# second-state/qwen3_asr_rs

Hardware: NVIDIA H100
Metric: real-time factor (audio-sec/wall-sec) Qwen3-ASR-0.6B 30s clips (higher is better)
Workload: dtype f32 (bf16 weights, fp32-exact activations)

## Files before the change

qwen3_asr_rs_b200/csrc/decode_batch.cu:

```cuda
#include <algorithm>
#include "mega_common.cuh"

namespace asrb {

namespace megab {
using namespace mega;

static constexpr int MAXSPLIT = 32;
static constexpr int MAXROWS = 8;
static constexpr int ATT_SCRATCH = 4 * HD + NCONS_WARPS * 2 * HD + NCONS_WARPS * 4 + 8 + 8 + 2 * HD;

struct Params {
    const DecLayerW* layers;
    const bf16* lm_head;
    const bf16* embed;
    const float* final_norm;
    const float* rope_cos; const float* rope_sin;
    float eps;
    int L, H, QD, KVD, I, V, nkv;
    int nb;
    float* x;
    float* kcache; float* vcache; size_t cache_layer_stride, cache_seq_stride; int max_ctx;
    float* part_val; int* part_idx; int n_part;
    int* pos; int* done; int* next_id; int* ids_out; int* n_out; int max_new;
// ... 46 lines not shown
            const uint32_t xrow = xp + (uint32_t)sq * (H * 2) + (uint32_t)swz16(xc0 + 2 * ks + bhalf, sq & 7) * 16u;
            uint32_t b00, b01, b10, b11, b20, b21;
            ldsm_x4(xrow + (uint32_t)bpl * PSTR, b00, b01, b10, b11);
            ldsm_x2(xrow + 2u * PSTR, b20, b21);
            mma16816(acc[nt], a0, a1, a2, a3, b00, b01);
            mma16816(acc1[nt], a0, a1, a2, a3, b10, b11);
            mma16816(acc2[nt], a0, a1, a2, a3, b20, b21);
        }
    }
#pragma unroll
    for (int nt = 0; nt < NT; ++nt)
#pragma unroll
        for (int k = 0; k < 4; ++k) acc[nt][k] += acc1[nt][k] + acc2[nt][k];
}

static constexpr uint32_t SX_EMPTY = 0xFFFFFFFFu;
__device__ __forceinline__ void sx_store(uint32_t* p, float v) {
    uint32_t b = __float_as_uint(v);
    if (b == SX_EMPTY) b = 0x7FFFFFFFu;
    asm volatile("red.relaxed.gpu.global.and.b32 [%0], %1;" ::"l"(p), "r"(b) : "memory");
}
__device__ __forceinline__ uint4 sx_load4(const uint32_t* p) {
    uint4 v;
    asm volatile("ld.relaxed.gpu.global.v4.u32 {%0, %1, %2, %3}, [%4];" : "=r"(v.x), "=r"(v.y), "=r"(v.z), "=r"(v.w) : "l"(p) : "memory");
    return v;
}

__device__ __forceinline__ void head_norm_rope_b(const uint2* __restrict__ src, uint32_t tag, const float* __restrict__ nw,
                                                 float eps, const float* __restrict__ cs, const float* __restrict__ sn,
                                                 float* dst, int lane) {
    float v[4];
    ll_poll4(src + lane, 32, tag, v);
    const float ss = warp_sum(v[0] * v[0] + v[1] * v[1] + v[2] * v[2] + v[3] * v[3]);
    const float r = 1.0f / sqrtf(ss / 128.f + eps);
#pragma unroll
    for (int i = 0; i < 4; ++i) v[i] = (v[i] * r) * __ldg(nw + lane + 32 * i);
#pragma unroll
    for (int i = 0; i < 2; ++i) {
        const int d = lane + 32 * i;
        const float c = cs[d], s = sn[d];
        const float a = v[i], b = v[i + 2];
// ... 755 lines not shown
```

qwen3_asr_rs_b200/csrc/decode_mega.cu:

```cuda
#include "mega_common.cuh"

namespace asrb {

namespace mega {

struct Params {
    const DecLayerW* layers;
    const bf16* lm_head;
    const bf16* embed;
    const float* final_norm;
    const float* rope_cos; const float* rope_sin;
    float eps;
    int L, H, QD, KVD, I, V, nq, nkv, group;
    float* x;
    float* kcache; float* vcache; size_t cache_layer_stride; int max_ctx;
    int nsplit;
    float* part_val; int* part_idx;
    int* pos; int* done; int* next_id; int* ids_out; int* n_out; int max_new;
    unsigned* bar;
    uint2* qkv_ll; uint2* part_ll; uint2* attn_ll; uint2* x_ll; uint2* act_ll;
    long long* dbg;
};

static_assert(KV_KEYS * HD * 4 == SLOT_BYTES, "K / V tiles travel through the weight ring: one tile per slot");

template <int K>
__device__ __forceinline__ void load_xr(const float* xs, float (&xr)[K / 32], int lane) {
    const int sw = ((lane >> 2) & 1) * 4;
#pragma unroll
    for (int c = 0; c < K / 256; ++c) {
        const float4 a = *reinterpret_cast<const float4*>(xs + (c * 32 + lane) * 8 + sw);
        const float4 b = *reinterpret_cast<const float4*>(xs + (c * 32 + lane) * 8 + 4 - sw);
        xr[c * 8 + 0] = a.x; xr[c * 8 + 1] = a.y; xr[c * 8 + 2] = a.z; xr[c * 8 + 3] = a.w;
        xr[c * 8 + 4] = b.x; xr[c * 8 + 5] = b.y; xr[c * 8 + 6] = b.z; xr[c * 8 + 7] = b.w;
    }
// ... 94 lines not shown
}

__device__ __forceinline__ float warp_reduce8(const float (&a)[8], int lane) {
    const bool h16 = lane & 16, h8 = lane & 8, h4 = lane & 4;
    float k[4];
#pragma unroll
    for (int i = 0; i < 4; ++i) k[i] = (h16 ? a[4 + i] : a[i]) + __shfl_xor_sync(0xffffffffu, h16 ? a[i] : a[4 + i], 16);
    float m0 = (h8 ? k[2] : k[0]) + __shfl_xor_sync(0xffffffffu, h8 ? k[0] : k[2], 8);
    float m1 = (h8 ? k[3] : k[1]) + __shfl_xor_sync(0xffffffffu, h8 ? k[1] : k[3], 8);
    float v = (h4 ? m1 : m0) + __shfl_xor_sync(0xffffffffu, h4 ? m0 : m1, 4);
    v += __shfl_xor_sync(0xffffffffu, v, 2);
    v += __shfl_xor_sync(0xffffffffu, v, 1);
    return v;
}

enum { ME_STORE = 0, ME_RESID = 1, ME_SWIGLU = 2, ME_ARGMAX = 3 };

template <int K>
__device__ __forceinline__ void consume_ksplit(const Slice& s, const Ring& ring, uint32_t& q, const float* xs, uint2* out,
                                               uint32_t tag, float* xres, float* part) {
    const int tid = threadIdx.x, lane = tid & 31, warp = tid >> 5;
    constexpr int NU = K / 8;
    constexpr int J = (NU + NCONS - 1) / NCONS;
    uint32_t grp = 0;
    for (int r = s.r0; r < s.r1;) {
        const int rowsA = min(s.rpc, s.r1 - r);
        const uint32_t slotA = q % ring.nslot;
        mbar_wait(&ring.full[slotA], (q / ring.nslot) & 1);
        const bool pair = s.rpc < 8 && r + rowsA < s.r1;
        const int rowsB = pair ? min(s.rpc, s.r1 - r - rowsA) : 0;
        const uint32_t slotB = (q + 1) % ring.nslot;
        if (pair) mbar_wait(&ring.full[slotB], ((q + 1) / ring.nslot) & 1);
        const uint4* baseA = reinterpret_cast<const uint4*>(ring.slots + (size_t)slotA * SLOT_BYTES);
        const uint4* baseB = reinterpret_cast<const uint4*>(ring.slots + (size_t)slotB * SLOT_BYTES);
        const int R = rowsA + rowsB;
// ... 29 lines not shown
            }
            const float v = warp_reduce8(acc, lane);
            if (g0 + 8 >= R) {
                __syncwarp();
                if (lane == 0) { mbar_arrive(&ring.empty[slotA]); if (pair) mbar_arrive(&ring.empty[slotB]); }
            }
            float* pb = part + (grp & 1) * 64;
            if ((lane & 3) == 0) pb[warp * 8 + (lane >> 2)] = v;
            cons_sync();
            if (tid < ng) {
                float t = pb[tid];
#pragma unroll
                for (int w8 = 1; w8 < NCONS_WARPS; ++w8) t += pb[w8 * 8 + tid];
                const int row = r + g0 + tid;
                const float nv = xres[row - s.r0] + t; xres[row - s.r0] = nv;
                ll_store(out + row, nv, tag);
            }
        }
        r += R; q += pair ? 2 : 1;
    }
}

template <int K, int EPI>
__device__ __forceinline__ void consume_quad(const Slice& s, const Ring& ring, uint32_t& q, const float* xs, uint2* out,
                                             uint32_t tag, float& best_v, int& best_i,
                                             const float* norm_w, float norm_r, long long* fine) {
    const int lane = threadIdx.x & 31, warp = threadIdx.x >> 5;
    int fi = 0;
#define CF() do { if (fine && threadIdx.x == 0 && fi < 24) fine[fi++] = clock64(); } while (0)
    CF();
    constexpr int NU = K / 8;
    float xr[K / 32];
    if (norm_w) load_xr_norm<K>(xs, norm_w, norm_r, xr, lane);
    else load_xr<K>(xs, xr, lane);
    cons_sync();
    CF();
    const int j = lane >> 3;
    for (int r = s.r0; r < s.r1;) {
        const int rowsA = min(s.rpc, s.r1 - r);
// ... 7 lines not shown
        const uint4* baseA = reinterpret_cast<const uint4*>(ring.slots + (size_t)slotA * SLOT_BYTES);
        const uint4* baseB = reinterpret_cast<const uint4*>(ring.slots + (size_t)slotB * SLOT_BYTES);
        const int R = rowsA + rowsB;
        for (int i0 = 4 * warp; i0 < R; i0 += 4 * NCONS_WARPS) {
            const int nv = min(4, R - i0);
            const uint4* rp[4];
#pragma unroll
            for (int i = 0; i < 4; ++i) {
                const int ri = i0 + (i < nv ? i : 0);
                rp[i] = ri < rowsA ? baseA + (size_t)ri * NU : baseB + (size_t)(ri - rowsA) * NU;
            }
            const float v = row_dot4<K>(rp[0], rp[1], rp[2], rp[3], xr, lane);
            const int row = r + i0 + j;
            if (EPI == ME_SWIGLU) {
                const float up = __shfl_xor_sync(0xffffffffu, v, 8);
                if ((lane & 15) == 0 && j < nv) ll_store(out + (row >> 1), silu(v) * up, tag);
            } else if (EPI == ME_STORE) {
                if ((lane & 7) == 0 && j < nv) ll_store(out + row, v, tag);
            } else {
                if ((lane & 7) == 0 && j < nv && v > best_v) { best_v = v; best_i = row; }
            }
        }
        CF();
        __syncwarp();
        if (lane == 0) { mbar_arrive(&ring.empty[slotA]); if (pair) mbar_arrive(&ring.empty[slotB]); }
        r += R; q += pair ? 2 : 1;
    }
    CF();
#undef CF
}

template <int K, int EPI>
__device__ __forceinline__ void consume(const Slice& s, const Ring& ring, uint32_t& q, const float* xs, uint2* out,
                                        uint32_t tag, float* xres, float& best_v, int& best_i,
                                        const float* norm_w = nullptr, float norm_r = 1.f, long long* fine = nullptr,
                                        float* part = nullptr) {
    if constexpr (EPI == ME_RESID) { consume_ksplit<K>(s, ring, q, xs, out, tag, xres, part); return; }
    else if constexpr (K <= 1024) { consume_quad<K, EPI>(s, ring, q, xs, out, tag, best_v, best_i, norm_w, norm_r, fine); return; }
    const int lane = threadIdx.x & 31, warp = threadIdx.x >> 5;
    int fi = 0;
#define CF() do { if (fine && threadIdx.x == 0 && fi < 24) fine[fi++] = clock64(); } while (0)
    CF();
    constexpr int RSTEP = (EPI == ME_SWIGLU) ? 2 : 1;
    constexpr bool XREG = K <= 2048;
    constexpr bool DUAL = XREG && K <= 1024;
    constexpr int KX = XREG ? K : 256;
    constexpr int UPW = (DUAL && EPI != ME_SWIGLU) ? 2 : 1;
    const int sub = lane >> 4;
    float xr[XREG ? K / 32 : 1];
    if (XREG) {
        if (norm_w) load_xr_norm<KX>(xs, norm_w, norm_r, reinterpret_cast<float (&)[KX / 32]>(xr), lane);
        else load_xr<KX>(xs, reinterpret_cast<float (&)[KX / 32]>(xr), lane);
        cons_sync();
// ... 11 lines not shown
        for (int ub = first * UPW; ub < units_here; ub += NCONS_WARPS * UPW) {
            if (EPI == ME_SWIGLU) {
                const int row = r + ub * 2;
                float v0, v1;
                if (DUAL) {
                    const float v = row_dot2<KX>(base + (size_t)(ub * 2) * (K / 8), base + (size_t)(ub * 2 + 1) * (K / 8),
                                                 reinterpret_cast<const float (&)[KX / 32]>(xr), lane);
                    v0 = v; v1 = __shfl_xor_sync(0xffffffffu, v, 16);
                } else if (XREG) {
                    v0 = row_dot<KX>(base + (size_t)(ub * 2) * (K / 8), reinterpret_cast<const float (&)[KX / 32]>(xr), lane);
                    v1 = row_dot<KX>(base + (size_t)(ub * 2 + 1) * (K / 8), reinterpret_cast<const float (&)[KX / 32]>(xr), lane);
                } else {
                    v0 = row_dot_smem<K>(base + (size_t)(ub * 2) * (K / 8), xs, lane);
                    v1 = row_dot_smem<K>(base + (size_t)(ub * 2 + 1) * (K / 8), xs, lane);
                }
                if (lane == 0) ll_store(out + (row >> 1), silu(v0) * v1, tag);
            } else {
                bool act; int row; float v0;
                if (DUAL) {
                    const bool two = ub + 1 < units_here;
                    v0 = row_dot2<KX>(base + (size_t)ub * (K / 8), base + (size_t)(two ? ub + 1 : ub) * (K / 8),
                                      reinterpret_cast<const float (&)[KX / 32]>(xr), lane);
                    act = ((lane & 15) == 0) && (sub == 0 || two);
                    row = r + ub + sub;
                } else {
                    if (XREG) v0 = row_dot<KX>(base + (size_t)ub * (K / 8), reinterpret_cast<const float (&)[KX / 32]>(xr), lane);
                    else v0 = row_dot_smem<K>(base + (size_t)ub * (K / 8), xs, lane);
                    act = lane == 0; row = r + ub;
                }
                if (EPI == ME_STORE) {
                    if (act) ll_store(out + row, v0, tag);
                } else if (EPI == ME_RESID) {
                    if (act) { const float nv = xres[row - s.r0] + v0; xres[row - s.r0] = nv; ll_store(out + row, nv, tag); }
                } else {
                    if (act && v0 > best_v) { best_v = v0; best_i = row; }
                }
            }
        }
        unit += (units_here + UPW - 1) / UPW * UPW;
        CF();
        __syncwarp();
        if (lane == 0) mbar_arrive(&ring.empty[slot]);
    }
    CF();
#undef CF
    if (!XREG) cons_sync();
}

// ... 34 lines not shown
#define MEGA_GT(k)                                                                                     \
    do {                                                                                               \
        if (p.dbg && tid == 0 && l == 5) {                                                             \
            unsigned long long t_; asm volatile("mov.u64 %0, %%globaltimer;" : "=l"(t_));               \
            p.dbg[512 + 3 * blockIdx.x + (k)] = (long long)t_;                                         \
        }                                                                                              \
    } while (0)
#define MEGA_MARK()                                                                                    \
    do {                                                                                               \
        if (dbg_row && tid == 0 && dbg_i < DBG_SLOTS) dbg_row[dbg_i++] = clock64();                    \
    } while (0)

template <int H, int QD, int I, int NS>
__global__ void __launch_bounds__(NTHREADS, 1) decode_step_kernel(const Params p) {
    constexpr int XS_FLOATS = (I > XS_MIN ? I : XS_MIN) + 64;
    extern __shared__ __align__(128) uint8_t smem[];
    constexpr int PARAM_FLOATS = 2 * H + 2 * HD;
    Ring ring;
    ring.slots = smem;
    ring.nslot = NS;
    float* xs = reinterpret_cast<float*>(smem + (size_t)NS * SLOT_BYTES);
    float* xres = xs + XS_FLOATS;
    float* pbuf = xres + XRES_MAX;
    float* ropes = pbuf + 2 * PARAM_FLOATS;
    DecLayerW* ltab = reinterpret_cast<DecLayerW*>(ropes + 128);
    uint64_t* bars = reinterpret_cast<uint64_t*>(ltab + MAX_LAYERS);
    ring.full = bars; ring.empty = bars + NSLOT_MAX;
    uint64_t* p_full = bars + 2 * NSLOT_MAX; uint64_t* p_empty = p_full + 2;
    float* red = reinterpret_cast<float*>(bars + 2 * NSLOT_MAX + 4);
    int* ired = reinterpret_cast<int*>(red + 64);
// ... 71 lines not shown

    long long* dbg_row = nullptr; int dbg_i = 0;
    if (p.dbg && (blockIdx.x == 0 || blockIdx.x == gridDim.x - 1)) dbg_row = p.dbg + (blockIdx.x == 0 ? 0 : DBG_SLOTS);
    MEGA_MARK();
    const int half = HD / 2;
    const float* cs = ropes;
    const float* sn = ropes + half;
    const unsigned G = gridDim.x;
    float best_v = -INFINITY; int best_i = 0x7fffffff;
    const unsigned epoch = __ldcg(p.bar + 1);
    const uint32_t tag_base = (epoch & 0xffffffu) << 8;
    const Slice xsl = make_slice(nullptr, H, QD, 1);
    Slice sl_qkv = make_slice(nullptr, QD + 2 * p.KVD, H, 1), sl_o = make_slice(nullptr, H, QD, 1),
          sl_gu = make_slice(nullptr, 2 * I, H, 2), sl_dn = make_slice(nullptr, H, I, 1);
    for (int i = tid; i < xsl.r1 - xsl.r0; i += NCONS) xres[i] = __ldcg(p.x + xsl.r0 + i);

    for (int l = 0; l < p.L; ++l) {
        const DecLayerW w = ltab[l];
        const uint32_t tl = tag_base | ((uint32_t)l << 3);
        const float* pb = pbuf + (l & 1) * PARAM_FLOATS;
        mbar_wait(&p_full[l & 1], (l >> 1) & 1);
        float nr;
        {
            float ss = 0.f;
            if (l == 0) { for (int i = tid; i < H; i += NCONS) { const float v = __ldcg(p.x + i); xs[xs_swz(i)] = v; ss = fmaf(v, v, ss); } }
            else { MEGA_FINE(0); MEGA_FINE(1); ss = ll_gather(p.x_ll, H, (tag_base | ((uint32_t)(l - 1) << 3)) | PH_XD, xs); MEGA_FINE(2); }
            nr = norm_scale(ss, H, p.eps, red);
            MEGA_FINE(3);
        }
        consume<H, ME_STORE>(sl_qkv, ring, q, xs, p.qkv_ll, tl | PH_QKV, xres, best_v, best_i, pb, nr);
        MEGA_FINE(4);
        MEGA_GT(0);
        MEGA_MARK();
        {
            const int nloc = n_old;
            const int nact = min(p.nsplit, (pos + KV_KEYS - 1) / KV_KEYS);
            const bool merger = att_cta && att_sp == 0;
            if (nloc > 0) {
                const int g = att_g;
                float* qs = xs;
                float* kn = qs + p.group * HD;
                float* vn = kn + HD;
                float* sc = vn + HD;
                float* ml = sc + p.group * KV_KEYS;
                float* osum = ml + 8;
// ... 176 lines not shown
                            ok = __all_sync(0xffffffffu, (mv.y == tg) && (lv.y == tg) && round_ok(0));
                        } while (!ok);
                        MEGA_FINE(35);
                        const float m_l = lane < nact ? __uint_as_float(mv.x) : (lane == nact ? snew[hq] : -INFINITY);
                        const float l_l = lane < nact ? __uint_as_float(lv.x) : (lane == nact ? 1.f : 0.f);
                        const float M = warp_max(m_l);
                        const float f = expf(m_l - M);
                        const float Lsum = warp_sum(f * l_l);
                        float O = __shfl_sync(0xffffffffu, f, nact) * vn[d];
                        for (int u0 = 0; u0 < nact; u0 += RB) {
                            if (u0 > 0) { do { load_round(u0); ok = __all_sync(0xffffffffu, round_ok(u0)); } while (!ok); }
#pragma unroll
                            for (int u = 0; u < RB; ++u)
                                if (u0 + u < nact) O = fmaf(__shfl_sync(0xffffffffu, f, u0 + u), __uint_as_float(ov[u].x), O);
                        }
                        ll_store(p.attn_ll + (size_t)(g * p.group + hq) * HD + d, O / Lsum, tl | PH_ATTN);
                    }
                }
                MEGA_FINE(31);
                cons_sync();
            }
        }
        MEGA_MARK();
        MEGA_FINE(32);
        ll_gather(p.attn_ll, QD, tl | PH_ATTN, xs);
        MEGA_FINE(33);
        MEGA_GT(2);
        cons_sync();
        consume<QD, ME_RESID>(sl_o, ring, q, xs, p.x_ll, tl | PH_XO, xres, best_v, best_i, nullptr, 1.f, nullptr, part);
        MEGA_FINE(34);
        MEGA_MARK();
        cons_sync();
        {
            MEGA_FINE(8); MEGA_FINE(9);
            const float ss = ll_gather(p.x_ll, H, tl | PH_XO, xs); MEGA_FINE(10);
            nr = norm_scale(ss, H, p.eps, red); MEGA_FINE(11);
        }
        consume<H, ME_SWIGLU>(sl_gu, ring, q, xs, p.act_ll, tl | PH_ACT, xres, best_v, best_i, pb + H, nr, (dbg_row && l == 5) ? dbg_row + 440 : nullptr);
        MEGA_FINE(12);
        MEGA_FINE(13);
        MEGA_MARK();
        MEGA_FINE(16); MEGA_FINE(17);
        ll_gather(p.act_ll, I, tl | PH_ACT, xs); MEGA_FINE(18);
        cons_sync();
        consume<I, ME_RESID>(sl_dn, ring, q, xs, p.x_ll, tl | PH_XD, xres, best_v, best_i, nullptr, 1.f, nullptr, part);
        MEGA_FINE(19);
        MEGA_FINE(20);
        MEGA_MARK();
        cons_sync();
        if (lane == 0) mbar_arrive(&p_empty[l & 1]);
    }
    float nrf;
    {
        const float ss = ll_gather(p.x_ll, H, (tag_base | ((uint32_t)(p.L - 1) << 3)) | PH_XD, xs);
        mbar_wait(&p_full[p.L & 1], (p.L >> 1) & 1);
        nrf = norm_scale(ss, H, p.eps, red);
    }
    consume<H, ME_ARGMAX>(make_slice(p.lm_head, p.V, H, 1), ring, q, xs, nullptr, 0u, xres, best_v, best_i,
                          pbuf + (p.L & 1) * PARAM_FLOATS, nrf);
    MEGA_MARK();
#pragma unroll
    for (int o = 8; o <= 16; o <<= 1) {
        const float ov = __shfl_xor_sync(0xffffffffu, best_v, o); const int oi = __shfl_xor_sync(0xffffffffu, best_i, o);
        if (ov > best_v || (ov == best_v && oi < best_i)) { best_v = ov; best_i = oi; }
    }
    cons_sync();
    if (lane == 0) { red[warp] = best_v; ired[warp] = best_i; }
    cons_sync();
    int& is_last = ired[63];
    if (tid == 0) {
        float v = -INFINITY; int idx = 0x7fffffff;
        for (int wq = 0; wq < NCONS_WARPS; ++wq)
            if (red[wq] > v || (red[wq] == v && ired[wq] < idx)) { v = red[wq]; idx = ired[wq]; }
// ... 17 lines not shown
            if (ov > v || (ov == v && oi < idx)) { v = ov; idx = oi; }
        }
        if (lane == 0) { red[warp] = v; ired[warp] = idx; }
        cons_sync();
        int& tok_s = ired[62];
        if (tid == 0) {
            for (int wq = 1; wq < NCONS_WARPS; ++wq)
                if (red[wq] > v || (red[wq] == v && ired[wq] < idx)) { v = red[wq]; idx = ired[wq]; }
            int tok = idx;
            const int n = *p.n_out;
            if (tok == 151643 || tok == 151645 || n >= p.max_new) { *p.done = 1; *p.next_id = -1; tok = -1; }
            else { p.ids_out[n] = tok; *p.n_out = n + 1; *p.pos = pos + 1; *p.next_id = tok; }
            tok_s = tok;
            p.bar[0] = 0;
            p.bar[1] = p.bar[1] + 1;
        }
        cons_sync();
        const int tok = tok_s;
        if (tok >= 0) {
            const bf16* e = p.embed + (size_t)tok * H;
            for (int i = tid; i < H; i += NCONS) p.x[i] = __bfloat162float(e[i]);
        }
    }
}

}

static long long* g_last_dbg = nullptr;

static int mega_xs_floats(int I) { return std::max(I, mega::XS_MIN) + 64; }
// ... 14 lines not shown
    if (B < 1 || c.head_dim != 128) return false;
    const int group = c.num_attention_heads / c.num_key_value_heads;
    if (group + 2 > mega::NCONS_WARPS) return false;
    if ((size_t)(group * 128 + 256 + group * mega::KV_KEYS + 8 + mega::NCONS_WARPS * 2 * 128 + mega::NCONS_WARPS * 4 + 8) > (size_t)mega_xs_floats(c.intermediate_size)) return false;
    if (m.ctx->smem_optin < mega_smem_bytes(c.hidden_size, c.intermediate_size, mega_nslot(c))) return false;
    if ((c.hidden_size + m.ctx->sm_count - 1) / m.ctx->sm_count + 1 > mega::XRES_MAX) return false;
    if (c.num_hidden_layers > 32) return false;
    if ((max_ctx + mega::KV_KEYS - 1) / mega::KV_KEYS > mega::MAX_SPLITS) return false;
    if (((max_ctx + mega::KV_KEYS - 1) / mega::KV_KEYS) * c.num_key_value_heads > m.ctx->sm_count) return false;
    return dims_match<1024, 2048, 3072>(c) || dims_match<2048, 2048, 6144>(c) || dims_match<256, 512, 512>(c);
}

size_t decode_mega_part_floats(const Model& m) {
    const asrb_dims& c = m.d.c;
    const int group = c.num_attention_heads / c.num_key_value_heads;
    const size_t words = (size_t)m.d.qkv_dim + (size_t)m.ctx->sm_count * group * mega::PSTRIDE + m.d.q_dim + c.hidden_size +
                         c.intermediate_size + 64;
    return 2 * words + 64;
}

void launch_decode_step_mega(const Model& m, const DecodeBufs& b, int B, float* kcache, float* vcache,
                             size_t cache_layer_stride, size_t cache_seq_stride, int max_ctx, int ctx_now, const MegaBufs& mb,
                             cudaStream_t st, int64_t* launches) {
    ASRB_REQUIRE(decode_mega_supported(m, B, ctx_now), ASRB_ERR_STATE, "fused decode step not supported for this model/batch/context");
    ASRB_REQUIRE(m.d_dec_layers && mb.bar && mb.part, ASRB_ERR_STATE, "fused decode step buffers missing");
    const asrb_dims& c = m.d.c;
    const int G = m.ctx->sm_count;
    const int group = c.num_attention_heads / c.num_key_value_heads;
    const int nsplit = std::min(mega::MAX_SPLITS, std::min(G / c.num_key_value_heads, (max_ctx + mega::KV_KEYS - 1) / mega::KV_KEYS));
    const size_t smem = mega_smem_bytes(c.hidden_size, c.intermediate_size, mega_nslot(c));
    const void* fn = nullptr;
    if (dims_match<1024, 2048, 3072>(c)) fn = (const void*)mega::decode_step_kernel<1024, 2048, 3072, 6>;
    else if (dims_match<2048, 2048, 6144>(c)) fn = (const void*)mega::decode_step_kernel<2048, 2048, 6144, 5>;
    else fn = (const void*)mega::decode_step_kernel<256, 512, 512, 6>;
    ASRB_CUDA_CHECK(cudaFuncSetAttribute(fn, cudaFuncAttributeMaxDynamicSharedMemorySize, (int)smem));
    for (int sb = 0; sb < B; ++sb) {
        mega::Params p{};
        p.layers = m.d_dec_layers; p.lm_head = m.lm_head; p.embed = m.embed; p.final_norm = m.final_norm_sw;
        p.rope_cos = m.rope_cos; p.rope_sin = m.rope_sin; p.eps = (float)c.rms_norm_eps;
        p.L = c.num_hidden_layers; p.H = c.hidden_size; p.QD = m.d.q_dim; p.KVD = m.d.kv_dim; p.I = c.intermediate_size;
        p.V = c.vocab_size; p.nq = c.num_attention_heads; p.nkv = c.num_key_value_heads; p.group = group;
        p.x = b.x + (size_t)sb * c.hidden_size;
        p.kcache = kcache + (size_t)sb * cache_seq_stride; p.vcache = vcache + (size_t)sb * cache_seq_stride;
        p.cache_layer_stride = cache_layer_stride; p.max_ctx = max_ctx; p.nsplit = nsplit;
        p.part_val = b.part_val; p.part_idx = b.part_idx;
        p.pos = b.pos + sb; p.done = b.done + sb; p.next_id = b.next_id + sb;
        p.ids_out = b.ids_out + (size_t)sb * b.max_new; p.n_out = b.n_out + sb; p.max_new = b.max_new;
        p.bar = mb.bar;
        uint2* w = reinterpret_cast<uint2*>(mb.part);
        p.qkv_ll = w; w += m.d.qkv_dim;
        p.part_ll = w; w += (size_t)G * group * mega::PSTRIDE;
        p.attn_ll = w; w += m.d.q_dim;
        p.x_ll = w; w += c.hidden_size;
        p.act_ll = w; w += c.intermediate_size;
        p.dbg = mb.dbg;
        g_last_dbg = mb.dbg;
        if (mb.steps_issued && ++*mb.steps_issued >= 0xFFFF00u) {
            ASRB_CUDA_CHECK(cudaMemsetAsync(mb.part, 0, mb.part_bytes, st));
            const unsigned one = 1;
            ASRB_CUDA_CHECK(cudaMemcpyAsync(mb.bar + 1, &one, sizeof(one), cudaMemcpyHostToDevice, st));
            *mb.steps_issued = 1;
        }
        void* args[] = {(void*)&p};
        ASRB_CUDA_CHECK(cudaLaunchCooperativeKernel(fn, dim3(G), dim3(mega::NTHREADS), args, smem, st));
        if (launches) *launches += 1;
    }
}

int decode_mega_debug_timeline(long long* out, int cap) {
// ... 9 lines not shown
```

qwen3_asr_rs_b200/csrc/internal.h:

```cpp
#pragma once
#include <atomic>
#include <map>
#include <string>
#include <vector>
#include "../../include/asr_b200.h"
#include "common.cuh"

namespace asrb {

struct Dims {
    asrb_dims c;
    int enc_hd;
    int chunk_frames;
    int chunks_per_window;
    int conv_h[4];
    int conv_w[4];
    int tok_per_chunk;
    int cpad;
    int feat;
    int q_dim, kv_dim, qkv_dim;
    void derive();
};
void validate_dims(const asrb_dims& d);
inline int conv_out_len(int l) { return (l - 1) / 2 + 1; }
// ... 121 lines not shown
    float* attn;
    float* act;
    float* logits;
    float* part_val; int* part_idx; int n_part;
    int* pos;
    int* done;
    int* next_id;
    int* ids_out;
    int* n_out;
    int max_new;
};
void launch_decode_step_phases(const Model& m, const DecodeBufs& b, int B, float* kcache, float* vcache,
                               size_t cache_layer_stride, size_t cache_seq_stride, int max_ctx,
                               bool write_logits, cudaStream_t st, int64_t* launches);
struct MegaBufs { unsigned* bar = nullptr; float* part = nullptr; long long* dbg = nullptr; size_t part_bytes = 0; unsigned* steps_issued = nullptr;
                  uint32_t* sx = nullptr; size_t sx_bytes = 0; int* sx_nb = nullptr; };
size_t decode_mega_part_floats(const Model& m);
size_t decode_batch_part_floats(const Model& m);
size_t decode_batch_sx_bytes(const Model& m);
bool decode_batch_supported(const Model& m, int B, int ctx);
int decode_mega_dbg_slots();
void launch_greedy(const Model& m, const DecodeBufs& b, int B, cudaStream_t st, int64_t* launches);
void launch_lmhead_argmax(const Model& m, const float* x_rows, const int* d_row_idx, int B,
                          const DecodeBufs& b, bool write_logits, cudaStream_t st, int64_t* launches);

}
```

qwen3_asr_rs_b200/csrc/mega_common.cuh:

```cuda
#pragma once
#include "internal.h"

namespace asrb {
namespace mega {

static constexpr int NCONS_WARPS = 8;
static constexpr int NCONS = NCONS_WARPS * 32;
static constexpr int NTHREADS = NCONS + 32;
static constexpr int SLOT_BYTES = 32 * 1024;
static constexpr int NSLOT_MAX = 6;
static constexpr int KV_KEYS = 64;
static constexpr int XS_MIN = 3072;
static constexpr int XRES_MAX = 64;
static constexpr int MAX_LAYERS = 32;
static constexpr int HD = 128;
static constexpr int PSTRIDE = HD + 2;
static constexpr int DBG_SLOTS = 1024;
static constexpr int MAX_SPLITS = 18;

enum { PH_QKV = 1, PH_PART = 2, PH_ATTN = 3, PH_XO = 4, PH_ACT = 5, PH_XD = 6 };

__device__ __forceinline__ uint32_t smem_u32(const void* p) { return (uint32_t)__cvta_generic_to_shared(p); }
__device__ __forceinline__ void mbar_init(uint64_t* bar, uint32_t count) {
    asm volatile("mbarrier.init.shared::cta.b64 [%0], %1;" ::"r"(smem_u32(bar)), "r"(count));
}
__device__ __forceinline__ void mbar_expect_tx(uint64_t* bar, uint32_t bytes) {
    asm volatile("mbarrier.arrive.expect_tx.shared::cta.b64 _, [%0], %1;" ::"r"(smem_u32(bar)), "r"(bytes) : "memory");
}
__device__ __forceinline__ void mbar_arrive(uint64_t* bar) {
    asm volatile("mbarrier.arrive.shared::cta.b64 _, [%0];" ::"r"(smem_u32(bar)) : "memory");
}
__device__ __forceinline__ void mbar_wait(uint64_t* bar, uint32_t parity) {
    asm volatile(
        "{\n"
        ".reg .pred p;\n"
// ... 11 lines not shown
__device__ __forceinline__ uint64_t l2_evict_first_policy() {
    uint64_t pol;
    asm volatile("createpolicy.fractional.L2::evict_first.b64 %0, 1.0;" : "=l"(pol));
    return pol;
}
__device__ __forceinline__ void bulk_g2s_hint(void* dst, const void* src, uint32_t bytes, uint64_t* bar, uint64_t pol) {
    asm volatile("cp.async.bulk.shared::cluster.global.mbarrier::complete_tx::bytes.L2::cache_hint [%0], [%1], %2, [%3], %4;"
                 ::"r"(smem_u32(dst)), "l"(src), "r"(bytes), "r"(smem_u32(bar)), "l"(pol) : "memory");
}
__device__ __forceinline__ void cons_sync() { asm volatile("bar.sync 1, %0;" ::"n"(NCONS) : "memory"); }

__device__ __forceinline__ void ll_store(uint2* p, float v, uint32_t tag) {
    const unsigned long long val = ((unsigned long long)tag << 32) | (unsigned long long)__float_as_uint(v);
    asm volatile("red.relaxed.gpu.global.max.u64 [%0], %1;" ::"l"(p), "l"(val) : "memory");
}
__device__ __forceinline__ uint4 ll_load2(const uint2* p) {
    uint4 v;
    asm volatile("ld.relaxed.gpu.global.v4.u32 {%0, %1, %2, %3}, [%4];" : "=r"(v.x), "=r"(v.y), "=r"(v.z), "=r"(v.w) : "l"(p) : "memory");
    return v;
}
__device__ __forceinline__ float ll_poll1(const uint2* p, uint32_t tag) {
    uint2 v;
    do {
        asm volatile("ld.relaxed.gpu.global.v2.u32 {%0, %1}, [%2];" : "=r"(v.x), "=r"(v.y) : "l"(p) : "memory");
    } while (v.y != tag);
    return __uint_as_float(v.x);
}
__device__ __forceinline__ void ll_poll4(const uint2* p, int stride, uint32_t tag, float (&out)[4]) {
    uint2 v[4];
    bool ok;
    do {
#pragma unroll
        for (int i = 0; i < 4; ++i)
            asm volatile("ld.relaxed.gpu.global.v2.u32 {%0, %1}, [%2];" : "=r"(v[i].x), "=r"(v[i].y) : "l"(p + (size_t)i * stride) : "memory");
        ok = (v[0].y == tag) && (v[1].y == tag) && (v[2].y == tag) && (v[3].y == tag);
    } while (!ok);
#pragma unroll
    for (int i = 0; i < 4; ++i) out[i] = __uint_as_float(v[i].x);
}
__device__ __forceinline__ int xs_swz(int e) { const int k = e >> 2; return ((k ^ ((k >> 3) & 1)) << 2) | (e & 3); }
__device__ __forceinline__ float ll_gather(const uint2* buf, int n, uint32_t tag, float* xs) {
    float ss = 0.f;
    const int pairs = n >> 1;
    constexpr int U = 8;
    for (int i0 = threadIdx.x; i0 < pairs; i0 += U * NCONS) {
        uint4 v[U];
#pragma unroll
        for (int u = 0; u < U; ++u) v[u] = make_uint4(0u, 0u, 0u, 0u);
        bool ok;
        do {
            ok = true;
#pragma unroll
            for (int u = 0; u < U; ++u) {
                const int i = i0 + u * NCONS;
                if (i < pairs && !(v[u].y == tag && v[u].w == tag)) v[u] = ll_load2(buf + 2 * i);
            }
#pragma unroll
            for (int u = 0; u < U; ++u) {
                const int i = i0 + u * NCONS;
                if (i < pairs) ok = ok && (v[u].y == tag) && (v[u].w == tag);
            }
        } while (!ok);
#pragma unroll
        for (int u = 0; u < U; ++u) {
            const int i = i0 + u * NCONS;
            if (i < pairs) {
                const float a = __uint_as_float(v[u].x), b = __uint_as_float(v[u].z);
                *reinterpret_cast<float2*>(xs + xs_swz(2 * i)) = make_float2(a, b);
                ss = fmaf(a, a, ss); ss = fmaf(b, b, ss);
            }
        }
    }
    return ss;
}

struct Ring {
    uint8_t* slots; uint64_t* full; uint64_t* empty;
    uint32_t nslot;
};

struct Slice { const bf16* W; int K, r0, r1, rpc; };
__device__ __forceinline__ Slice make_slice(const bf16* W, int N, int K, int rstep) {
// ... 12 lines not shown
```

qwen3_asr_rs_b200/csrc/session.cu:

```cuda
#include <algorithm>
#include <cstring>
#include "internal.h"

namespace asrb {

void model_set_tensor(Model* m, const char* name, int dtype, const int64_t* shape, int ndim, const void* host);
void model_finalize(Model* m);
struct IngestState;
IngestState* ingest_state_new();
void ingest_state_free(IngestState* st);
void ingest_pcm(IngestState* st, cudaStream_t stream, const void* const* pcm, const int64_t* n_frames, const int32_t* channels,
                const int32_t* rate, const int32_t* format, int batch, float* d_samples, int64_t max_samples_per_utt,
                int64_t* n_out, int64_t* soff_out);

static const int kPromptHead[9] = {151644, 8948, 198, 151645, 198, 151644, 872, 198, 151669};
static const int kPromptTail[6] = {151670, 151645, 198, 151644, 77091, 198};
static const int kAudioPad = 151676;

struct Session {
    Model* m = nullptr;
    cudaStream_t st = nullptr;
    int max_batch = 0, max_lang = 0, max_new = 0;
    int64_t max_samples = 0, max_npad = 0;
    int maxF = 0, maxC = 0, maxT = 0, maxS = 0, max_ctx = 0;
// ... 126 lines not shown
        b.act = salloc<float>(s, Bm * c.intermediate_size);
        b.logits = salloc<float>(s, Bm * c.vocab_size);
        b.n_part = m->ctx->sm_count * 2;
        b.part_val = salloc<float>(s, Bm * b.n_part);
        b.part_idx = salloc<int>(s, Bm * b.n_part);
        b.pos = salloc<int>(s, Bm); b.done = salloc<int>(s, Bm); b.next_id = salloc<int>(s, Bm);
        b.ids_out = salloc<int>(s, Bm * max_new); b.n_out = salloc<int>(s, Bm);
        b.max_new = max_new;
        s->d_lastrow = salloc<int>(s, Bm);
        s->mega.bar = salloc<unsigned>(s, 4, true);
        { const unsigned one = 1; ASRB_CUDA_CHECK(cudaMemcpy(s->mega.bar + 1, &one, sizeof(one), cudaMemcpyHostToDevice)); }
        const size_t part_floats = std::max(decode_mega_part_floats(*m), decode_batch_part_floats(*m));
        s->mega.part = salloc<float>(s, part_floats, true);
        s->mega.part_bytes = part_floats * sizeof(float);
        s->mega.steps_issued = &s->mega_steps;
        if (max_batch >= 2) {
            s->mega.sx_bytes = decode_batch_sx_bytes(*m);
            s->mega.sx = (uint32_t*)salloc<uint8_t>(s, s->mega.sx_bytes);
            ASRB_CUDA_CHECK(cudaMemset(s->mega.sx, 0xFF, s->mega.sx_bytes));
            s->mega.sx_nb = &s->sx_nb;
            int maxwin = 0, maxpersist = 0;
            cudaDeviceGetAttribute(&maxwin, cudaDevAttrMaxAccessPolicyWindowSize, m->ctx->device);
            cudaDeviceGetAttribute(&maxpersist, cudaDevAttrMaxPersistingL2CacheSize, m->ctx->device);
            if (maxwin > 0 && maxpersist > 0) {
                const size_t want = std::min<size_t>({s->mega.sx_bytes, (size_t)maxwin, (size_t)maxpersist});
                if (cudaDeviceSetLimit(cudaLimitPersistingL2CacheSize, want) == cudaSuccess) {
                    cudaStreamAttrValue av{};
                    av.accessPolicyWindow.base_ptr = s->mega.sx; av.accessPolicyWindow.num_bytes = want;
                    av.accessPolicyWindow.hitRatio = 1.0f; av.accessPolicyWindow.hitProp = cudaAccessPropertyPersisting;
                    av.accessPolicyWindow.missProp = cudaAccessPropertyStreaming;
// ... 429 lines not shown
```

Before: 294.6.

## Replace tagged LL buffers in single-sequence mega decode with per-layer sentinel exchange buffers

The single-sequence fused decode kernel stops exchanging attention output, residual and activations through tagged 64-bit LL slots. It now uses per-layer, double-buffered 32-bit sentinel buffers (all-ones means empty) that are filled with atomic AND and polled with vectorized relaxed loads. Because the buffers are distinct per layer, several cons_sync barriers between phases are removed, and the k-split residual now writes straight into these buffers. Each step clears the other parity's buffers, which adds global stores. The exchange also halves its traffic per value and uses a new gather pattern, optionally as a noinline call when H > 1024.

```diff
diff --git a/qwen3_asr_rs_b200/csrc/decode_batch.cu b/qwen3_asr_rs_b200/csrc/decode_batch.cu
--- a/qwen3_asr_rs_b200/csrc/decode_batch.cu
+++ b/qwen3_asr_rs_b200/csrc/decode_batch.cu
@@ -84,17 +84,6 @@
         for (int k = 0; k < 4; ++k) acc[nt][k] += acc1[nt][k] + acc2[nt][k];
 }
 
-static constexpr uint32_t SX_EMPTY = 0xFFFFFFFFu;
-__device__ __forceinline__ void sx_store(uint32_t* p, float v) {
-    uint32_t b = __float_as_uint(v);
-    if (b == SX_EMPTY) b = 0x7FFFFFFFu;
-    asm volatile("red.relaxed.gpu.global.and.b32 [%0], %1;" ::"l"(p), "r"(b) : "memory");
-}
-__device__ __forceinline__ uint4 sx_load4(const uint32_t* p) {
-    uint4 v;
-    asm volatile("ld.relaxed.gpu.global.v4.u32 {%0, %1, %2, %3}, [%4];" : "=r"(v.x), "=r"(v.y), "=r"(v.z), "=r"(v.w) : "l"(p) : "memory");
-    return v;
-}
 
 __device__ __forceinline__ void head_norm_rope_b(const uint2* __restrict__ src, uint32_t tag, const float* __restrict__ nw,
                                                  float eps, const float* __restrict__ cs, const float* __restrict__ sn,
diff --git a/qwen3_asr_rs_b200/csrc/decode_mega.cu b/qwen3_asr_rs_b200/csrc/decode_mega.cu
--- a/qwen3_asr_rs_b200/csrc/decode_mega.cu
+++ b/qwen3_asr_rs_b200/csrc/decode_mega.cu
@@ -18,7 +18,8 @@
     float* part_val; int* part_idx;
     int* pos; int* done; int* next_id; int* ids_out; int* n_out; int max_new;
     unsigned* bar;
-    uint2* qkv_ll; uint2* part_ll; uint2* attn_ll; uint2* x_ll; uint2* act_ll;
+    uint2* qkv_ll; uint2* part_ll;
+    uint32_t* sx;
     long long* dbg;
 };
 
@@ -143,11 +144,56 @@
     return v;
 }
 
-enum { ME_STORE = 0, ME_RESID = 1, ME_SWIGLU = 2, ME_ARGMAX = 3 };
+enum { ME_STORE = 0, ME_SWIGLU = 2, ME_ARGMAX = 3 };
+
+__device__ __forceinline__ void publish(uint2* p, float v, uint32_t tag) { ll_store(p, v, tag); }
+__device__ __forceinline__ void publish(uint32_t* p, float v, uint32_t) { sx_store(p, v); }
 
 template <int K>
-__device__ __forceinline__ void consume_ksplit(const Slice& s, const Ring& ring, uint32_t& q, const float* xs, uint2* out,
-                                               uint32_t tag, float* xres, float* part) {
+__device__ __forceinline__ void ksplit_gather(const uint32_t* src, float* xs) {
+    constexpr int Q = K / 4;
+    constexpr int QW = (Q + 2 * NCONS - 1) / (2 * NCONS);
+    constexpr int BB = QW < 2 ? QW : 2;
+    const int lane = threadIdx.x & 31, warp = threadIdx.x >> 5;
+#pragma unroll
+    for (int b0 = 0; b0 < QW; b0 += BB) {
+        uint4 v[2 * BB];
+#pragma unroll
+        for (int u = 0; u < 2 * BB; ++u) v[u] = make_uint4(SX_EMPTY, SX_EMPTY, SX_EMPTY, SX_EMPTY);
+        auto quad = [&](int u) __attribute__((always_inline)) { return (b0 + (u >> 1)) * 2 * NCONS + warp * 64 + (u & 1) * 32 + lane; };
+        bool ok;
+        do {
+            ok = true;
+#pragma unroll
+            for (int u = 0; u < 2 * BB; ++u)
+                if (b0 + (u >> 1) < QW && quad(u) < Q && !sx_ready4(v[u])) v[u] = sx_load4(src + 4 * quad(u));
+#pragma unroll
+            for (int u = 0; u < 2 * BB; ++u)
+                if (b0 + (u >> 1) < QW && quad(u) < Q) ok = ok && sx_ready4(v[u]);
+        } while (!ok);
+#pragma unroll
+        for (int u = 0; u < 2 * BB; ++u) {
+            const int k = quad(u);
+            if (b0 + (u >> 1) < QW && k < Q)
+                *reinterpret_cast<float4*>(xs + 4 * (k ^ ((k >> 3) & 1))) =
+                    make_float4(__uint_as_float(v[u].x), __uint_as_float(v[u].y), __uint_as_float(v[u].z), __uint_as_float(v[u].w));
+        }
+    }
+    __syncwarp();
+}
+
+template <int K> __device__ __noinline__ void ksplit_gather_call(const uint32_t* src, float* xs) { ksplit_gather<K>(src, xs); }
+__device__ __noinline__ float sx_gather_call(const uint32_t* buf, int n, float* xs) { return sx_gather(buf, n, xs); }
+template <bool CALL, int K> __device__ __forceinline__ void ksplit_gather_sel(const uint32_t* src, float* xs) {
+    if constexpr (CALL) ksplit_gather_call<K>(src, xs); else ksplit_gather<K>(src, xs);
+}
+template <bool CALL> __device__ __forceinline__ float sx_gather_sel(const uint32_t* buf, int n, float* xs) {
+    if constexpr (CALL) return sx_gather_call(buf, n, xs); else return sx_gather(buf, n, xs);
+}
+
+template <int K>
+__device__ __forceinline__ void consume_ksplit(const Slice& s, const Ring& ring, uint32_t& q, const float* xs, uint32_t* out,
+                                               float* xres, float* part) {
     const int tid = threadIdx.x, lane = tid & 31, warp = tid >> 5;
     constexpr int NU = K / 8;
     constexpr int J = (NU + NCONS - 1) / NCONS;
@@ -207,15 +253,15 @@
                 for (int w8 = 1; w8 < NCONS_WARPS; ++w8) t += pb[w8 * 8 + tid];
                 const int row = r + g0 + tid;
                 const float nv = xres[row - s.r0] + t; xres[row - s.r0] = nv;
-                ll_store(out + row, nv, tag);
+                sx_store(out + row, nv);
             }
         }
         r += R; q += pair ? 2 : 1;
     }
 }
 
-template <int K, int EPI>
-__device__ __forceinline__ void consume_quad(const Slice& s, const Ring& ring, uint32_t& q, const float* xs, uint2* out,
+template <int K, int EPI, typename Out>
+__device__ __forceinline__ void consume_quad(const Slice& s, const Ring& ring, uint32_t& q, const float* xs, Out* out,
                                              uint32_t tag, float& best_v, int& best_i,
                                              const float* norm_w, float norm_r, long long* fine) {
     const int lane = threadIdx.x & 31, warp = threadIdx.x >> 5;
@@ -253,9 +299,9 @@
             const int row = r + i0 + j;
             if (EPI == ME_SWIGLU) {
                 const float up = __shfl_xor_sync(0xffffffffu, v, 8);
-                if ((lane & 15) == 0 && j < nv) ll_store(out + (row >> 1), silu(v) * up, tag);
+                if ((lane & 15) == 0 && j < nv) publish(out + (row >> 1), silu(v) * up, tag);
             } else if (EPI == ME_STORE) {
-                if ((lane & 7) == 0 && j < nv) ll_store(out + row, v, tag);
+                if ((lane & 7) == 0 && j < nv) publish(out + row, v, tag);
             } else {
                 if ((lane & 7) == 0 && j < nv && v > best_v) { best_v = v; best_i = row; }
             }
@@ -269,13 +315,11 @@
 #undef CF
 }
 
-template <int K, int EPI>
-__device__ __forceinline__ void consume(const Slice& s, const Ring& ring, uint32_t& q, const float* xs, uint2* out,
-                                        uint32_t tag, float* xres, float& best_v, int& best_i,
-                                        const float* norm_w = nullptr, float norm_r = 1.f, long long* fine = nullptr,
-                                        float* part = nullptr) {
-    if constexpr (EPI == ME_RESID) { consume_ksplit<K>(s, ring, q, xs, out, tag, xres, part); return; }
-    else if constexpr (K <= 1024) { consume_quad<K, EPI>(s, ring, q, xs, out, tag, best_v, best_i, norm_w, norm_r, fine); return; }
+template <int K, int EPI, typename Out>
+__device__ __forceinline__ void consume(const Slice& s, const Ring& ring, uint32_t& q, const float* xs, Out* out,
+                                        uint32_t tag, float& best_v, int& best_i,
+                                        const float* norm_w = nullptr, float norm_r = 1.f, long long* fine = nullptr) {
+    if constexpr (K <= 1024) { consume_quad<K, EPI>(s, ring, q, xs, out, tag, best_v, best_i, norm_w, norm_r, fine); return; }
     const int lane = threadIdx.x & 31, warp = threadIdx.x >> 5;
     int fi = 0;
 #define CF() do { if (fine && threadIdx.x == 0 && fi < 24) fine[fi++] = clock64(); } while (0)
@@ -317,7 +361,7 @@
                     v0 = row_dot_smem<K>(base + (size_t)(ub * 2) * (K / 8), xs, lane);
                     v1 = row_dot_smem<K>(base + (size_t)(ub * 2 + 1) * (K / 8), xs, lane);
                 }
-                if (lane == 0) ll_store(out + (row >> 1), silu(v0) * v1, tag);
+                if (lane == 0) publish(out + (row >> 1), silu(v0) * v1, tag);
             } else {
                 bool act; int row; float v0;
                 if (DUAL) {
@@ -332,9 +376,7 @@
                     act = lane == 0; row = r + ub;
                 }
                 if (EPI == ME_STORE) {
-                    if (act) ll_store(out + row, v0, tag);
-                } else if (EPI == ME_RESID) {
-                    if (act) { const float nv = xres[row - s.r0] + v0; xres[row - s.r0] = nv; ll_store(out + row, nv, tag); }
+                    if (act) publish(out + row, v0, tag);
                 } else {
                     if (act && v0 > best_v) { best_v = v0; best_i = row; }
                 }
@@ -399,6 +441,7 @@
 template <int H, int QD, int I, int NS>
 __global__ void __launch_bounds__(NTHREADS, 1) decode_step_kernel(const Params p) {
     constexpr int XS_FLOATS = (I > XS_MIN ? I : XS_MIN) + 64;
+    constexpr bool GCALL = H > 1024;
     extern __shared__ __align__(128) uint8_t smem[];
     constexpr int PARAM_FLOATS = 2 * H + 2 * HD;
     Ring ring;
@@ -500,6 +543,16 @@
     Slice sl_qkv = make_slice(nullptr, QD + 2 * p.KVD, H, 1), sl_o = make_slice(nullptr, H, QD, 1),
           sl_gu = make_slice(nullptr, 2 * I, H, 2), sl_dn = make_slice(nullptr, H, I, 1);
     for (int i = tid; i < xsl.r1 - xsl.r0; i += NCONS) xres[i] = __ldcg(p.x + xsl.r0 + i);
+    constexpr size_t SX_LAYER = (size_t)2 * H + QD + I;
+    const unsigned sstep = __ldcg(p.bar + 3);
+    const int sx_l0 = (int)(sstep & 1u) * p.L;
+    auto sx_at = [&](int l, int off) __attribute__((always_inline)) { return p.sx + (size_t)(sx_l0 + l) * SX_LAYER + off; };
+    {
+        uint4* const other = reinterpret_cast<uint4*>(p.sx + (size_t)((sstep & 1u) ^ 1u) * p.L * SX_LAYER);
+        const unsigned nq = (unsigned)(p.L * SX_LAYER / 4);
+        const unsigned q0 = blockIdx.x * nq / G, q1 = (blockIdx.x + 1) * nq / G;
+        for (unsigned i = q0 + tid; i < q1; i += NCONS) other[i] = make_uint4(SX_EMPTY, SX_EMPTY, SX_EMPTY, SX_EMPTY);
+    }
 
     for (int l = 0; l < p.L; ++l) {
         const DecLayerW w = ltab[l];
@@ -510,11 +563,11 @@
         {
             float ss = 0.f;
             if (l == 0) { for (int i = tid; i < H; i += NCONS) { const float v = __ldcg(p.x + i); xs[xs_swz(i)] = v; ss = fmaf(v, v, ss); } }
-            else { MEGA_FINE(0); MEGA_FINE(1); ss = ll_gather(p.x_ll, H, (tag_base | ((uint32_t)(l - 1) << 3)) | PH_XD, xs); MEGA_FINE(2); }
+            else { MEGA_FINE(0); MEGA_FINE(1); ss = sx_gather_sel<GCALL>(sx_at(l - 1, H), H, xs); MEGA_FINE(2); }
             nr = norm_scale(ss, H, p.eps, red);
             MEGA_FINE(3);
         }
-        consume<H, ME_STORE>(sl_qkv, ring, q, xs, p.qkv_ll, tl | PH_QKV, xres, best_v, best_i, pb, nr);
+        consume<H, ME_STORE>(sl_qkv, ring, q, xs, p.qkv_ll, tl | PH_QKV, best_v, best_i, pb, nr);
         MEGA_FINE(4);
         MEGA_GT(0);
         MEGA_MARK();
@@ -721,7 +774,7 @@
                             for (int u = 0; u < RB; ++u)
                                 if (u0 + u < nact) O = fmaf(__shfl_sync(0xffffffffu, f, u0 + u), __uint_as_float(ov[u].x), O);
                         }
-                        ll_store(p.attn_ll + (size_t)(g * p.group + hq) * HD + d, O / Lsum, tl | PH_ATTN);
+                        sx_store(sx_at(l, 2 * H) + (g * p.group + hq) * HD + d, O / Lsum);
                     }
                 }
                 MEGA_FINE(31);
@@ -730,27 +783,24 @@
         }
         MEGA_MARK();
         MEGA_FINE(32);
-        ll_gather(p.attn_ll, QD, tl | PH_ATTN, xs);
+        ksplit_gather_sel<GCALL, QD>(sx_at(l, 2 * H), xs);
         MEGA_FINE(33);
         MEGA_GT(2);
-        cons_sync();
-        consume<QD, ME_RESID>(sl_o, ring, q, xs, p.x_ll, tl | PH_XO, xres, best_v, best_i, nullptr, 1.f, nullptr, part);
+        consume_ksplit<QD>(sl_o, ring, q, xs, sx_at(l, 0), xres, part);
         MEGA_FINE(34);
         MEGA_MARK();
-        cons_sync();
         {
             MEGA_FINE(8); MEGA_FINE(9);
-            const float ss = ll_gather(p.x_ll, H, tl | PH_XO, xs); MEGA_FINE(10);
+            const float ss = sx_gather_sel<GCALL>(sx_at(l, 0), H, xs); MEGA_FINE(10);
             nr = norm_scale(ss, H, p.eps, red); MEGA_FINE(11);
         }
-        consume<H, ME_SWIGLU>(sl_gu, ring, q, xs, p.act_ll, tl | PH_ACT, xres, best_v, best_i, pb + H, nr, (dbg_row && l == 5) ? dbg_row + 440 : nullptr);
+        consume<H, ME_SWIGLU>(sl_gu, ring, q, xs, sx_at(l, 2 * H + QD), 0u, best_v, best_i, pb + H, nr, (dbg_row && l == 5) ? dbg_row + 440 : nullptr);
         MEGA_FINE(12);
         MEGA_FINE(13);
         MEGA_MARK();
         MEGA_FINE(16); MEGA_FINE(17);
-        ll_gather(p.act_ll, I, tl | PH_ACT, xs); MEGA_FINE(18);
-        cons_sync();
-        consume<I, ME_RESID>(sl_dn, ring, q, xs, p.x_ll, tl | PH_XD, xres, best_v, best_i, nullptr, 1.f, nullptr, part);
+        ksplit_gather_sel<GCALL, I>(sx_at(l, 2 * H + QD), xs); MEGA_FINE(18);
+        consume_ksplit<I>(sl_dn, ring, q, xs, sx_at(l, H), xres, part);
         MEGA_FINE(19);
         MEGA_FINE(20);
         MEGA_MARK();
@@ -759,11 +809,11 @@
     }
     float nrf;
     {
-        const float ss = ll_gather(p.x_ll, H, (tag_base | ((uint32_t)(p.L - 1) << 3)) | PH_XD, xs);
+        const float ss = sx_gather_sel<GCALL>(sx_at(p.L - 1, H), H, xs);
         mbar_wait(&p_full[p.L & 1], (p.L >> 1) & 1);
         nrf = norm_scale(ss, H, p.eps, red);
     }
-    consume<H, ME_ARGMAX>(make_slice(p.lm_head, p.V, H, 1), ring, q, xs, nullptr, 0u, xres, best_v, best_i,
+    consume<H, ME_ARGMAX>(make_slice(p.lm_head, p.V, H, 1), ring, q, xs, static_cast<uint32_t*>(nullptr), 0u, best_v, best_i,
                           pbuf + (p.L & 1) * PARAM_FLOATS, nrf);
     MEGA_MARK();
 #pragma unroll
@@ -811,6 +861,7 @@
             tok_s = tok;
             p.bar[0] = 0;
             p.bar[1] = p.bar[1] + 1;
+            p.bar[3] = p.bar[3] + 1;
         }
         cons_sync();
         const int tok = tok_s;
@@ -855,16 +906,19 @@
 size_t decode_mega_part_floats(const Model& m) {
     const asrb_dims& c = m.d.c;
     const int group = c.num_attention_heads / c.num_key_value_heads;
-    const size_t words = (size_t)m.d.qkv_dim + (size_t)m.ctx->sm_count * group * mega::PSTRIDE + m.d.q_dim + c.hidden_size +
-                         c.intermediate_size + 64;
+    const size_t words = (size_t)m.d.qkv_dim + (size_t)m.ctx->sm_count * group * mega::PSTRIDE + 64;
     return 2 * words + 64;
+}
+size_t decode_mega_sx_bytes(const Model& m) {
+    const asrb_dims& c = m.d.c;
+    return (size_t)2 * c.num_hidden_layers * ((size_t)2 * c.hidden_size + m.d.q_dim + c.intermediate_size) * 4;
 }
 
 void launch_decode_step_mega(const Model& m, const DecodeBufs& b, int B, float* kcache, float* vcache,
                              size_t cache_layer_stride, size_t cache_seq_stride, int max_ctx, int ctx_now, const MegaBufs& mb,
                              cudaStream_t st, int64_t* launches) {
     ASRB_REQUIRE(decode_mega_supported(m, B, ctx_now), ASRB_ERR_STATE, "fused decode step not supported for this model/batch/context");
-    ASRB_REQUIRE(m.d_dec_layers && mb.bar && mb.part, ASRB_ERR_STATE, "fused decode step buffers missing");
+    ASRB_REQUIRE(m.d_dec_layers && mb.bar && mb.part && mb.seq_sx, ASRB_ERR_STATE, "fused decode step buffers missing");
     const asrb_dims& c = m.d.c;
     const int G = m.ctx->sm_count;
     const int group = c.num_attention_heads / c.num_key_value_heads;
@@ -890,10 +944,8 @@
         p.bar = mb.bar;
         uint2* w = reinterpret_cast<uint2*>(mb.part);
         p.qkv_ll = w; w += m.d.qkv_dim;
-        p.part_ll = w; w += (size_t)G * group * mega::PSTRIDE;
-        p.attn_ll = w; w += m.d.q_dim;
-        p.x_ll = w; w += c.hidden_size;
-        p.act_ll = w; w += c.intermediate_size;
+        p.part_ll = w;
+        p.sx = mb.seq_sx;
         p.dbg = mb.dbg;
         g_last_dbg = mb.dbg;
         if (mb.steps_issued && ++*mb.steps_issued >= 0xFFFF00u) {
diff --git a/qwen3_asr_rs_b200/csrc/internal.h b/qwen3_asr_rs_b200/csrc/internal.h
--- a/qwen3_asr_rs_b200/csrc/internal.h
+++ b/qwen3_asr_rs_b200/csrc/internal.h
@@ -159,8 +159,10 @@
                                size_t cache_layer_stride, size_t cache_seq_stride, int max_ctx,
                                bool write_logits, cudaStream_t st, int64_t* launches);
 struct MegaBufs { unsigned* bar = nullptr; float* part = nullptr; long long* dbg = nullptr; size_t part_bytes = 0; unsigned* steps_issued = nullptr;
+                  uint32_t* seq_sx = nullptr;
                   uint32_t* sx = nullptr; size_t sx_bytes = 0; int* sx_nb = nullptr; };
 size_t decode_mega_part_floats(const Model& m);
+size_t decode_mega_sx_bytes(const Model& m);
 size_t decode_batch_part_floats(const Model& m);
 size_t decode_batch_sx_bytes(const Model& m);
 bool decode_batch_supported(const Model& m, int B, int ctx);
diff --git a/qwen3_asr_rs_b200/csrc/mega_common.cuh b/qwen3_asr_rs_b200/csrc/mega_common.cuh
--- a/qwen3_asr_rs_b200/csrc/mega_common.cuh
+++ b/qwen3_asr_rs_b200/csrc/mega_common.cuh
@@ -18,7 +18,7 @@
 static constexpr int DBG_SLOTS = 1024;
 static constexpr int MAX_SPLITS = 18;
 
-enum { PH_QKV = 1, PH_PART = 2, PH_ATTN = 3, PH_XO = 4, PH_ACT = 5, PH_XD = 6 };
+enum { PH_QKV = 1, PH_PART = 2 };
 
 __device__ __forceinline__ uint32_t smem_u32(const void* p) { return (uint32_t)__cvta_generic_to_shared(p); }
 __device__ __forceinline__ void mbar_init(uint64_t* bar, uint32_t count) {
@@ -60,11 +60,6 @@
     const unsigned long long val = ((unsigned long long)tag << 32) | (unsigned long long)__float_as_uint(v);
     asm volatile("red.relaxed.gpu.global.max.u64 [%0], %1;" ::"l"(p), "l"(val) : "memory");
 }
-__device__ __forceinline__ uint4 ll_load2(const uint2* p) {
-    uint4 v;
-    asm volatile("ld.relaxed.gpu.global.v4.u32 {%0, %1, %2, %3}, [%4];" : "=r"(v.x), "=r"(v.y), "=r"(v.z), "=r"(v.w) : "l"(p) : "memory");
-    return v;
-}
 __device__ __forceinline__ float ll_poll1(const uint2* p, uint32_t tag) {
     uint2 v;
     do {
@@ -84,34 +79,55 @@
 #pragma unroll
     for (int i = 0; i < 4; ++i) out[i] = __uint_as_float(v[i].x);
 }
+
+static constexpr uint32_t SX_EMPTY = 0xFFFFFFFFu;
+__device__ __forceinline__ void sx_store(uint32_t* p, float v) {
+    uint32_t b = __float_as_uint(v);
+    if (b == SX_EMPTY) b = 0x7FFFFFFFu;
+    asm volatile("red.relaxed.gpu.global.and.b32 [%0], %1;" ::"l"(p), "r"(b) : "memory");
+}
+__device__ __forceinline__ uint4 sx_load4(const uint32_t* p) {
+    uint4 v;
+    asm volatile("ld.relaxed.gpu.global.v4.u32 {%0, %1, %2, %3}, [%4];" : "=r"(v.x), "=r"(v.y), "=r"(v.z), "=r"(v.w) : "l"(p) : "memory");
+    return v;
+}
+__device__ __forceinline__ bool sx_ready4(const uint4& v) {
+    return v.x != SX_EMPTY && v.y != SX_EMPTY && v.z != SX_EMPTY && v.w != SX_EMPTY;
+}
+__device__ __forceinline__ uint2 sx_load2(const uint32_t* p) {
+    uint2 v;
+    asm volatile("ld.relaxed.gpu.global.v2.u32 {%0, %1}, [%2];" : "=r"(v.x), "=r"(v.y) : "l"(p) : "memory");
+    return v;
+}
+
 __device__ __forceinline__ int xs_swz(int e) { const int k = e >> 2; return ((k ^ ((k >> 3) & 1)) << 2) | (e & 3); }
-__device__ __forceinline__ float ll_gather(const uint2* buf, int n, uint32_t tag, float* xs) {
+__device__ __forceinline__ float sx_gather(const uint32_t* buf, int n, float* xs) {
     float ss = 0.f;
     const int pairs = n >> 1;
     constexpr int U = 8;
     for (int i0 = threadIdx.x; i0 < pairs; i0 += U * NCONS) {
-        uint4 v[U];
+        uint2 v[U];
 #pragma unroll
-        for (int u = 0; u < U; ++u) v[u] = make_uint4(0u, 0u, 0u, 0u);
+        for (int u = 0; u < U; ++u) v[u] = make_uint2(SX_EMPTY, SX_EMPTY);
         bool ok;
         do {
             ok = true;
 #pragma unroll
             for (int u = 0; u < U; ++u) {
                 const int i = i0 + u * NCONS;
-                if (i < pairs && !(v[u].y == tag && v[u].w == tag)) v[u] = ll_load2(buf + 2 * i);
+                if (i < pairs && (v[u].x == SX_EMPTY || v[u].y == SX_EMPTY)) v[u] = sx_load2(buf + 2 * i);
             }
 #pragma unroll
             for (int u = 0; u < U; ++u) {
                 const int i = i0 + u * NCONS;
-                if (i < pairs) ok = ok && (v[u].y == tag) && (v[u].w == tag);
+                if (i < pairs) ok = ok && (v[u].x != SX_EMPTY) && (v[u].y != SX_EMPTY);
             }
         } while (!ok);
 #pragma unroll
         for (int u = 0; u < U; ++u) {
             const int i = i0 + u * NCONS;
             if (i < pairs) {
-                const float a = __uint_as_float(v[u].x), b = __uint_as_float(v[u].z);
+                const float a = __uint_as_float(v[u].x), b = __uint_as_float(v[u].y);
                 *reinterpret_cast<float2*>(xs + xs_swz(2 * i)) = make_float2(a, b);
                 ss = fmaf(a, a, ss); ss = fmaf(b, b, ss);
             }
diff --git a/qwen3_asr_rs_b200/csrc/session.cu b/qwen3_asr_rs_b200/csrc/session.cu
--- a/qwen3_asr_rs_b200/csrc/session.cu
+++ b/qwen3_asr_rs_b200/csrc/session.cu
@@ -164,6 +164,11 @@
         s->mega.part = salloc<float>(s, part_floats, true);
         s->mega.part_bytes = part_floats * sizeof(float);
         s->mega.steps_issued = &s->mega_steps;
+        {
+            const size_t bytes = decode_mega_sx_bytes(*m);
+            s->mega.seq_sx = (uint32_t*)salloc<uint8_t>(s, bytes);
+            ASRB_CUDA_CHECK(cudaMemset(s->mega.seq_sx, 0xFF, bytes));
+        }
         if (max_batch >= 2) {
             s->mega.sx_bytes = decode_batch_sx_bytes(*m);
             s->mega.sx = (uint32_t*)salloc<uint8_t>(s, s->mega.sx_bytes);
```

New measurement: 301.8 (median of 6 runs). +2.5%, better.
